# RoboSafe-Lab/Controllable-Latent-Diffusion-for-Traffic-Simulation

Hardware: NVIDIA B200
Metric: guided scenarios/sec (50-step DDIM) (higher is better)
Workload: dtype bf16

## Files before the change

controllable-latent-diffusion-for-traffic-simulation_b200/csrc/cld_api.cu:

```cuda
#include <math.h>
#include <stdarg.h>
#include <stdlib.h>
#include <string.h>

#include "common.cuh"
#include "unet_tc.cuh"

static std::string g_create_err;

namespace cld {

int fail(CldHandle* h, int code, const char* fmt, ...) {
  char buf[512];
  va_list ap;
  va_start(ap, fmt);
  vsnprintf(buf, sizeof(buf), fmt, ap);
  va_end(ap);
  if (h) h->err = buf; else g_create_err = buf;
  return code;
}

int prof_begin(CldHandle* h, int kind, cudaStream_t s) {
  if (!h->profiling) return 0;
  if (h->ev_used + 2 > h->ev_pool.size()) {
// ... 149 lines not shown
    block(2 * lvl + 1);
    if (lvl < 2) conv(u.down[lvl], c.dims[lvl], c.dims[lvl], 3, k3, L.down[lvl][0], L.down[lvl][1]);
  }
  for (int lvl = 0; lvl < 2; ++lvl) {
    block(8 + 2 * lvl);
    block(9 + 2 * lvl);
    const int ch = lvl == 0 ? d1 : d0;
    const int iw = L.up[lvl][0] = take((int64_t)ch * ch * 4), ib = L.up[lvl][1] = take(ch);
    pack(u.up[lvl][0], iw, ch, ch, 4, 2, kte, 1);
    pack(u.up[lvl][1], iw, ch, ch, 4, 2, kto, 1);
    job(2, ib, buf(&u.up_b[lvl], ch), ch);
  }
  block(6);
  block(7);
  conv(u.fin0, d0, d0, 5, k5, L.fin[0], L.fin[1]);
  L.fin[2] = vec(&u.fin0n.g, d0);
  L.fin[3] = vec(&u.fin0n.b, d0);
  conv(u.fin1, D, d0, 1, k1, L.fin[4], L.fin[5]);
  if (rc) return rc;
  if (L.numel.size() > (size_t)PACK_MAX_SRC)
    return fail(h, CLD_ERR_UNSUPPORTED, "the denoiser has %zu tensors, the weight pack takes at most %d", L.numel.size(), PACK_MAX_SRC);
  for (PackJob& j : jobs) {
    j.blk0 = h->pack_blocks;
    h->pack_blocks += (j.total + PACK_BLOCK_ELEMS - 1) / PACK_BLOCK_ELEMS;
  }
  h->pack_njobs = (int)jobs.size();
  if ((rc = dev_alloc(h, &h->pack_jobs, jobs.size()))) return rc;
  CLD_CUDA_OK(h, cudaMemcpy(h->pack_jobs, jobs.data(), jobs.size() * sizeof(PackJob), cudaMemcpyHostToDevice));
  CLD_CUDA_OK(h, cudaStreamSynchronize(cudaStreamLegacy));
  return 0;
}

}

using namespace cld;

extern "C" {

int cld_version(void) { return 100; }

const char* cld_last_error(const CldHandle* h) { return h ? h->err.c_str() : g_create_err.c_str(); }

int cld_create(const CldConfig* cfg, CldHandle** out) {
  if (!cfg || !out) return fail(nullptr, CLD_ERR_ARG, "null argument");
  *out = nullptr;
  int dev = 0;
  cudaError_t e = cudaGetDevice(&dev);
  if (e != cudaSuccess) return fail(nullptr, CLD_ERR_CUDA, "cudaGetDevice: %s", cudaGetErrorString(e));
  cudaDeviceProp prop;
  e = cudaGetDeviceProperties(&prop, dev);
  if (e != cudaSuccess) return fail(nullptr, CLD_ERR_CUDA, "cudaGetDeviceProperties: %s", cudaGetErrorString(e));
  if (prop.major != 10)
    return fail(nullptr, CLD_ERR_ARCH, "libcld_b200 requires an sm_100 (B200) device, found sm_%d%d; there is no fallback",
                prop.major, prop.minor);
  if (cfg->horizon % 4 || cfg->horizon < 8 || cfg->horizon > CLD_MAX_T)
    return fail(nullptr, CLD_ERR_ARG, "horizon must be a multiple of 4 in [8,%d]", CLD_MAX_T);
  if (cfg->latent_dim != 4) return fail(nullptr, CLD_ERR_UNSUPPORTED, "latent_dim must be 4");
  if (cfg->base_dim < 2 || cfg->base_dim > 64 || cfg->base_dim % 4)
    return fail(nullptr, CLD_ERR_UNSUPPORTED, "base_dim must be a multiple of 4 in [4,64]");
  for (int i = 0; i < 3; ++i)
    if (cfg->dims[i] % 8 || cfg->dims[i] < 8) return fail(nullptr, CLD_ERR_UNSUPPORTED, "dims must be multiples of 8");
  if (cfg->cond_dim % 4 || cfg->cond_dim < 4) return fail(nullptr, CLD_ERR_UNSUPPORTED, "cond_dim must be a multiple of 4");
  if (cfg->max_rows < 1) return fail(nullptr, CLD_ERR_ARG, "max_rows must be positive");
  if (cfg->n_timesteps < 1) return fail(nullptr, CLD_ERR_ARG, "n_timesteps must be positive");
  {
    TcLevel levels[3];
    const bool t_ok = tc_level_layout(cfg->horizon, levels);
    if (cfg->precision == CLD_PREC_BF16 && !(cfg->dims[0] == 64 && cfg->dims[1] == 128 && cfg->dims[2] == 256 && t_ok && cfg->hidden == 64))
      return fail(nullptr, CLD_ERR_UNSUPPORTED,
                  "the bf16 tensor-core path is built for dims (64,128,256), hidden 64 and a horizon of 16..56 (8 rows per CTA) or 64..104 in "
                  "multiples of 8 (4 rows per CTA as two half-horizon lanes); use precision fp32 for this configuration");
  }
  CldHandle* h = new CldHandle();
  h->cfg = *cfg;
  h->device = dev;
  h->num_sms = prop.multiProcessorCount;
  h->use_lstm_tc = cfg->precision == CLD_PREC_BF16 && cfg->hidden == 64 && getenv("CLD_LSTM_SIMT") == nullptr;
  h->env_lstm_bwd_simt = getenv("CLD_LSTM_BWD_SIMT") != nullptr;
  h->env_guidance_nofork = getenv("CLD_GUIDANCE_NOFORK") != nullptr;
  h->env_lstm_prof = getenv("CLD_LSTM_PROF") != nullptr;
  h->env_map_stats = getenv("CLD_MAP_STATS") != nullptr;
  h->env_map_exhaustive = getenv("CLD_MAP_EXHAUSTIVE") != nullptr;
  h->env_train_serial = getenv("CLD_TRAIN_SERIAL") != nullptr;
  if (const char* e = getenv("CLD_LSTM_PF")) h->env_lstm_pf = atoi(e);
  const int T = cfg->horizon;
  const size_t MR = cfg->max_rows;
  size_t ae = (size_t)T * cfg->dims[0];
  if ((size_t)(T / 2) * cfg->dims[1] > ae) ae = (size_t)(T / 2) * cfg->dims[1];
  if ((size_t)(T / 4) * cfg->dims[2] > ae) ae = (size_t)(T / 4) * cfg->dims[2];
  h->act_elems = ae;
  unet_blocks(h->unet, *cfg);
  const int tb_total = h->unet.tb_total;
  int rc = 0;
  for (int i = 0; i < 7 && !rc; ++i) rc = dev_alloc(h, &h->act[i], MR * ae);
  if (!rc) rc = dev_alloc(h, &h->tcm, MR * (cfg->base_dim + cfg->cond_dim));
  if (!rc) rc = dev_alloc(h, &h->tbias, MR * tb_total);
  if (!rc) rc = dev_alloc(h, &h->tvec, tb_total);
  if (!rc) rc = dev_alloc(h, &h->tvec_all, (size_t)cfg->n_timesteps * tb_total);
  if (!rc) rc = dev_alloc(h, &h->stash, (size_t)2 * T * ((MR + 63) / 64 * 64) * 5 * cfg->hidden);
  if (!rc) rc = dev_alloc(h, &h->ws_act, MR * T * 2);
  if (!rc) rc = dev_alloc(h, &h->ws_h0, MR * cfg->hidden);
  if (!rc) rc = dev_alloc(h, &h->ws_dh0, (size_t)T * MR * cfg->hidden);
  if (!rc) rc = dev_alloc(h, &h->ws_traj, MR * T * 6);
  if (!rc) rc = dev_alloc(h, &h->ws_dtraj, MR * T * 4);
  if (!rc && h->use_lstm_tc) rc = dev_alloc(h, &h->ws_dtraj2, MR * T * 4);
  if (!rc) rc = dev_alloc(h, &h->ws_dacc, MR * T);
  if (!rc) rc = dev_alloc(h, &h->map_work, MR * T + 8);
  if (!rc && cudaMemset(h->map_work, 0, 8 * sizeof(int)) != cudaSuccess) rc = fail(h, CLD_ERR_CUDA, "cudaMemset of the map work list failed");
  if (!rc) rc = dev_alloc(h, &h->ws_loss, 7 * MR);
  if (!rc) rc = dev_alloc(h, &h->ws_eps, MR * T * cfg->latent_dim);
  if (!rc) rc = dev_alloc(h, &h->ws_mean, MR * T * cfg->latent_dim);
  if (!rc) rc = dev_alloc(h, &h->ws_x, MR * T * cfg->latent_dim);
  if (!rc) rc = dev_alloc(h, &h->ws_t, MR);
  if (!rc) rc = unet_setup(h);
  if (rc) {
    g_create_err = h->err;
    cld_destroy(h);
    return rc;
  }
  *out = h;
  return CLD_OK;
}

void cld_destroy(CldHandle* h) {
  if (!h) return;
  tc_destroy(h);
  lstm_tc_destroy(h);
  train_destroy(h);
  train_tc_destroy(h);
  if (h->ev_fork) cudaEventDestroy(h->ev_fork);
  if (h->ev_join) cudaEventDestroy(h->ev_join);
  if (h->ev_tvec) cudaEventDestroy(h->ev_tvec);
  if (h->aux_stream) cudaStreamDestroy(h->aux_stream);
  for (cudaEvent_t e : h->ev_pool) cudaEventDestroy(e);
  for (void* p : h->allocs) cudaFree(p);
  delete h;
}

int cld_load_unet(CldHandle* h, const float* const* p, const int64_t* numels, int n, void* stream) {
  if (!h || !p) return fail(h, CLD_ERR_ARG, "null argument");
  const UnetLayout& L = h->unet_layout;
  if (n != (int)L.numel.size()) return fail(h, CLD_ERR_ARG, "cld_load_unet: expected %zu tensors, got %d", L.numel.size(), n);
  PackSrc src;
  for (int i = 0; i < n; ++i) {
    if (!p[i]) return fail(h, CLD_ERR_ARG, "cld_load_unet: tensor %d is null", i);
    if (numels && numels[i] != L.numel[i])
      return fail(h, CLD_ERR_ARG, "cld_load_unet: tensor %d has %lld elements, expected %lld", i, (long long)numels[i], (long long)L.numel[i]);
    src.p[i] = p[i];
  }
  cudaStream_t s = (cudaStream_t)stream;
  repack_all_kernel<<<h->pack_blocks, 256, 0, s>>>(h->pack_jobs, h->pack_njobs, src);
  CLD_LAUNCH_OK(h, "repack_all_kernel");
  h->tvec_all_valid = false;
  train_invalidate(h);
  int rc;
  if (h->cfg.precision == CLD_PREC_BF16 && (rc = tc_finalize(h, p, s))) return rc;
  h->unet.loaded = true;
  return CLD_OK;
}

int cld_load_decoder(CldHandle* h, const float* const* p, int n, void* stream) {
  if (!h || !p) return fail(h, CLD_ERR_ARG, "null argument");
  if (n != 12) return fail(h, CLD_ERR_ARG, "cld_load_decoder: expected 12 tensors, got %d", n);
  cudaStream_t s = (cudaStream_t)stream;
  const int H = h->cfg.hidden, G = 4 * H, C = h->cfg.cond_dim, D = h->cfg.latent_dim;
  DecoderW& w = h->dec;
  int rc;
// ... 391 lines not shown
```

controllable-latent-diffusion-for-traffic-simulation_b200/csrc/common.cuh:

```cuda
#pragma once
#include <cuda_runtime.h>
#include <cuda_bf16.h>
#include <stdint.h>
#include <stdio.h>
#include <string>
#include <vector>

#include "../../include/cld_b200.h"

#define CLD_MAX_T 128
#define CLD_TB_TOTAL_MAX 4096

namespace cld {

struct ConvW {
  float* w = nullptr;
  float* wt = nullptr;
  float* b = nullptr;
  int cin = 0, cout = 0, ntaps = 0;
};
struct GnW {
  float* g = nullptr;
  float* b = nullptr;
};
// ... 37 lines not shown
  bool loaded = false;
};

}

namespace cld {
struct BlkIdx { int tw, tb, c0w, c0b, g0, b0, c1w, c1b, g1, b1, rw, rb; };
struct UnetLayout {
  std::vector<int64_t> numel;
  int tmlp[4];
  BlkIdx blk[12];
  int down[2][2], up[2][2];
  int fin[6];
};

struct PackJob {
  int kind;
  int src;
  float* dst;
  int cout, cin, K, ntaps, ks[5], ld, off, transposed, total, blk0;
};
}

struct CldHandle {
  CldConfig cfg;
  int device = 0;
  int num_sms = 0;
  std::string err;
  cld::UnetW unet;
  cld::UnetLayout unet_layout;
  cld::DecoderW dec;
  cld::Schedule sched;
  std::vector<void*> allocs;
  float* act[8] = {nullptr};
  size_t act_elems = 0;
  float* tcm = nullptr;
  float* tbias = nullptr;
  float* tvec = nullptr;
  float* tvec_all = nullptr;
  bool tvec_all_valid = false;
  cudaEvent_t ev_tvec = nullptr;
  cudaStream_t tvec_stream = nullptr;
  float* stash = nullptr;
  float* ws_act = nullptr;
  float* ws_h0 = nullptr;
  float* ws_dh0 = nullptr;
  float* ws_traj = nullptr;
  float* ws_dtraj = nullptr;
  float* ws_dtraj2 = nullptr;
  float* ws_dacc = nullptr;
  float* ws_adam_m = nullptr;
  float* ws_adam_v = nullptr;
  int* map_work = nullptr;
  uint8_t* map_bits = nullptr;
  size_t map_bits_bytes = 0;
  const void* screen_src = nullptr;
  const uint8_t* screen_pk = nullptr;
  int screen_agents = 0, screen_h = 0, screen_w = 0, screen_packed = 0, screen_pitch = 0;
  cudaStream_t aux_stream = nullptr;
  cudaEvent_t ev_fork = nullptr, ev_join = nullptr;
  float* ws_loss = nullptr;
  float* ws_eps = nullptr;
  float* ws_mean = nullptr;
  float* ws_x = nullptr;
  int64_t* ws_t = nullptr;
  int dbg_stage = -1;
  float* dbg_out = nullptr;
  unsigned long long launches = 0;
  bool profiling = false;
  std::vector<cudaEvent_t> ev_pool;
  std::vector<int> ev_kind;
  size_t ev_used = 0;
  void* tc = nullptr;
  void* lstm_tc = nullptr;
  bool use_lstm_tc = false;
  void* train = nullptr;
  unsigned long long sched_version = 0;
  cld::PackJob* pack_jobs = nullptr;
  int pack_njobs = 0, pack_blocks = 0;
  void* train_tc = nullptr;
  bool train_tf32 = false;
  bool env_train_serial = false;
  bool env_lstm_bwd_simt = false, env_guidance_nofork = false, env_lstm_prof = false, env_map_stats = false, env_map_exhaustive = false;
  int env_lstm_pf = 3;
};

namespace cld {
__host__ __device__ inline size_t stash_index(int layer, int t, int T, int R, int row, int v, int u) {
  const size_t rblk = (size_t)((R + 63) >> 6) * 8;
  return (((((size_t)layer * T + t) * rblk + (size_t)(row >> 3)) * 5 + v) * 64 + u) * 8 + (row & 7);
}
constexpr int STASH_V_STRIDE = 64 * 8;
int fail(CldHandle* h, int code, const char* fmt, ...);
#define CLD_CUDA_OK(h, expr)                                                                   \
  do {                                                                                         \
    cudaError_t _e = (expr);                                                                   \
    if (_e != cudaSuccess)                                                                     \
      return cld::fail(h, CLD_ERR_CUDA, "%s failed: %s (%s:%d)", #expr, cudaGetErrorString(_e), \
                       __FILE__, __LINE__);                                                    \
  } while (0)
#define CLD_LAUNCH_OK(h, name)                                                             \
  do {                                                                                     \
    cudaError_t _e = cudaGetLastError();                                                   \
    if (_e != cudaSuccess)                                                                 \
      return cld::fail(h, CLD_ERR_CUDA, "launch of %s failed: %s", name, cudaGetErrorString(_e)); \
    if (h) ++(h)->launches;                                                                \
  } while (0)

int prof_begin(CldHandle* h, int kind, cudaStream_t s);
int prof_end(CldHandle* h, cudaStream_t s);
int unet_forward_fp32(CldHandle* h, const float* x, const float* cond, const int64_t* t, float* eps,
                      int R, cudaStream_t s);
int unet_stage_elems(const CldHandle* h, int stage);
int unet_time_bias(CldHandle* h, const float* cond, const int64_t* t, int R, cudaStream_t s);
int unet_time_cond(CldHandle* h, const float* cond, const int64_t* t, int R, cudaStream_t s);
int unet_cond_bias(CldHandle* h, const float* cond, int R, cudaStream_t s);
int unet_time_vec(CldHandle* h, int t, cudaStream_t s);
int unet_time_vec_to(CldHandle* h, int t, float* dst, cudaStream_t s);
int gn_mish_launch(CldHandle* h, const float* in, const GnW& n, const float* tbias, int tb_stride, const float* res, float* out,
                   int T, int C, int R, cudaStream_t s);
int unet_train_forward(CldHandle* h, const float* x, const float* cond, const int64_t* t, float* eps, int R, cudaStream_t s);
int unet_train_backward(CldHandle* h, const float* d_eps, float* const* grads, int n, float* dx_out, int R, cudaStream_t s);
int ppo_head(CldHandle* h, const float* eps, const float* x_t, const float* x_tm1, const int64_t* t, const float* logp_old,
             const float* reward, float baseline, const float* baseline_dev, float clip, float* logp_new, float* loss_out, float* d_eps, int R,
             cudaStream_t s);
int adam_step_dev(CldHandle* h, float* p, const float* g, float* m, float* v, size_t n, const double* lr_dev, long long* step_dev, double b1,
                  double b2, double eps, double wd, cudaStream_t s);
int mse_head(CldHandle* h, const float* eps, const float* noise, float* loss_out, float* d_eps, int R, cudaStream_t s);
int adam_step(CldHandle* h, float* p, const float* g, float* m, float* v, size_t n, double lr, double b1, double b2, double eps, double wd,
              int step, cudaStream_t s);
float* train_deps_buffer(CldHandle* h);
bool tfconv_supported(int c0, int c1, int N, int Tp);
int tfconv_launch(CldHandle* h, const float* in0, int c0, const float* in1, int c1, int Ta, int tstride, int Tp, const float* w, int planes,
                  int ntaps, const int* wtap, const int* toff, const float* bias, float* out, int Tout, int ostride, int ooff, int N, int accum,
                  int R, cudaStream_t s);
bool tfwgrad_supported(int c0, int c1, int cout, int Tp, int R);
int tfwgrad_launch(CldHandle* h, const float* in0, int c0, const float* in1, int c1, int Ta, int a_stride, int Tp, const float* dout, int Td,
                   int d_stride, int d_toff, int cout, int ntaps, const int* toff, float* part, size_t part_floats, int max_splits, int R,
                   int* splits_out, cudaStream_t s);
void train_tc_destroy(CldHandle* h);
void train_destroy(CldHandle* h);
void train_invalidate(CldHandle* h);
int posterior_step(CldHandle* h, const float* x, const float* eps, const float* noise, uint64_t seed,
                   uint64_t seq, uint64_t idx_base, int t, int t_next, int sampler, float* x_out, float* mean_out, int R,
                   cudaStream_t s);
int add_noise(CldHandle* h, const float* mean, const float* noise, uint64_t seed, uint64_t seq, uint64_t idx_base, int t,
              float* x_out, int R, cudaStream_t s);
int philox_fill(CldHandle* h, uint64_t seed, uint64_t seq, uint64_t idx_base, float* out, int R, cudaStream_t s);
int fill_t(CldHandle* h, int64_t* t, int value, int R, cudaStream_t s);
int decode_rollout(CldHandle* h, const float* z, const float* cond, const float* curr, float* act_out,
                   float* traj_out, bool save, int R, cudaStream_t s);
int unicycle(CldHandle* h, const float* curr, const float* u, float* state_out, int R, cudaStream_t s);
struct GuideOpt {
  int iter = 1;
  float* m = nullptr;
  float* v = nullptr;
  float step_size = 0.f;
  float bc2_sqrt = 0.f;
};
int decode_h0(CldHandle* h, const float* cond, float* h0, int R, cudaStream_t s);
int decode_backward_update2(CldHandle* h, const float* z_mean, const float* act, const float* curr, const float* dtraj,
                            const float* dtraj2, const float* dacc, const CldGuidanceConfig* g, const GuideOpt& opt, float* z_out,
                            float* grad_out, int R, cudaStream_t s);
int decode_rollout_h0(CldHandle* h, const float* z, const float* h0, const float* curr, float* act_out, float* traj_out,
                      bool save, int R, cudaStream_t s);
int decode_rollout_h0_tc(CldHandle* h, const float* z, const float* h0, const float* curr, float* act_out, float* traj_out,
                         bool save, int R, cudaStream_t s);
int decode_backward_update_tc(CldHandle* h, const float* z_mean, const float* act, const float* curr, const float* dtraj,
                              const float* dtraj2, const float* dacc, const CldGuidanceConfig* g, const GuideOpt& opt, float* z_out,
                              float* grad_out, int R, cudaStream_t s);
void lstm_tc_destroy(CldHandle* h);
int indicators(CldHandle* h, const float* traj, const CldScene* sc, uint8_t* offroad, float* coll,
               float* reward, int R, cudaStream_t s);
int guidance_loss_grad(CldHandle* h, const float* traj, const CldScene* sc, const CldGuidanceConfig* g,
                       float* dtraj, float* dtraj_map, float* dacc, float* loss, int R, cudaStream_t s);
int guidance_prepare_maps(CldHandle* h, const CldScene* sc, cudaStream_t s);
int decode_backward_update(CldHandle* h, const float* z_mean, const float* act, const float* curr,
                           const float* dtraj, const CldGuidanceConfig* g, float* z_out, float* grad_out,
                           int R, cudaStream_t s);
}
```

controllable-latent-diffusion-for-traffic-simulation_b200/csrc/kernels_lstm_tc.cu:

```cuda
#include <cuda_fp16.h>
#include <stdio.h>
#include <stdlib.h>

#include "common.cuh"
#include "lstm_shared.cuh"
#include "tc_common.cuh"

namespace cld {
using namespace tc;

namespace {
constexpr int LT_RB = 32;
constexpr int LT_H = 64;
constexpr int LT_THREADS = 576;
constexpr int LT_WBLK = 16384;
constexpr int LT_OP = 4096;
constexpr int LF_H0 = 0;
constexpr int LF_H1 = LF_H0 + 4 * LT_OP;
constexpr int LF_Z = LF_H1 + 2 * LT_OP;
constexpr int LF_H1F = LF_Z + 6 * LT_OP;
constexpr int LF_H1P = LT_H + 1;
constexpr int LF_HW = LF_H1F + 2 * LT_RB * LF_H1P * 4;
constexpr int LF_BARS = LF_HW + 2 * LT_H * 4;
constexpr int LF_TMEM = LF_BARS + 8 * 8;
// ... 308 lines not shown
        if (PROF && rec && n1a >= P0 && n1a < P0 + PN) tl[n1a - P0][2] = clock64();
        tc_fence_after();
        const uint32_t d1a = tmem_base + 64u + (uint32_t)((n1a & 1) * 64);
        const uint64_t b_1a = bh0 + (uint64_t)((n1a & 1) * 2 * (LT_OP >> 4));
        if (elect_one()) kblock(d1a, wc + 80u, 64u, b_1a, 4, true);
        __syncwarp();
        if (PROF && rec && n1a >= P0 && n1a < P0 + PN) tl[n1a - P0][3] = clock64();
        ++n1a; progressed = true;
      }
      if (!progressed && clock64() - t_loop > 8000000000ll) {
        if (lane == 0) printf("lstm_tc forward: MMA issuer stuck (block %d, n0 %d n1a %d n1b %d e0 %d e1 %d z %d)\n", (int)blockIdx.x, n0, n1a, n1b, e0_done, e1_done, z_done);
        __trap();
      }
    }
    if (PROF && rec)
      for (int k = 0; k < PN; ++k)
        printf("[fwd prof] mma step %d: M0 %7lld - %7lld | M1a %7lld - %7lld | M1b %7lld - %7lld\n", P0 + k, tl[k][0] - tbase, tl[k][1] - tbase,
               tl[k][2] - tbase, tl[k][3] - tbase, tl[k][4] - tbase, tl[k][5] - tbase);
  } else {
    const int row = row0 + lane;
    const bool valid = row < R;
    const float hb0 = a.h2a_b[0], hb1 = a.h2a_b[1];
    if (lane == 0) { mbar_arrive(bar_z); mbar_arrive(bar_z + 8); mbar_arrive(bar_z + 16); }
    float4 zn = make_float4(0.f, 0.f, 0.f, 0.f);
    if (valid && 3 < T) zn = reinterpret_cast<const float4*>(a.z)[(size_t)row * T + 3];
    const DynParams2& d = a.dyn;
    float px = 0.f, py = 0.f, sp = 0.f, psi = 0.f;
    if (valid) { px = a.curr[(size_t)row * 4 + 0]; py = a.curr[(size_t)row * 4 + 1]; sp = a.curr[(size_t)row * 4 + 2]; psi = a.curr[(size_t)row * 4 + 3]; }
    float vprev = clip2(sp, d.v_lo, d.v_hi);
    for (int s = 1; s <= T; ++s) {
      const int t = s - 1;
      lt_wait(bar_e1, (uint32_t)t & 1u, 20000 + t);
      const float* hf = h1f + (t & 1) * (LT_RB * LF_H1P) + lane * LF_H1P;
      float s0 = hb0, s1 = hb1;
#pragma unroll 16
      for (int k = 0; k < LT_H; ++k) {
        const float hv = hf[k];
        s0 = fmaf(hw[k], hv, s0); s1 = fmaf(hw[LT_H + k], hv, s1);
      }
      __syncwarp();
      if (lane == 0) mbar_arrive(bar_a);
      if (s + 2 < T) {
        const int slot = (s + 2) % 3;
        uint8_t* zt = sm + LF_Z + slot * 2 * LT_OP;
        store_split(zt, lane, 0, zn.x); store_split(zt, lane, 1, zn.y); store_split(zt, lane, 2, zn.z); store_split(zt, lane, 3, zn.w);
        fence_proxy_async();
        __syncwarp();
        if (lane == 0) mbar_arrive(bar_z + 8 * slot);
        zn = make_float4(0.f, 0.f, 0.f, 0.f);
        if (valid && s + 3 < T) zn = reinterpret_cast<const float4*>(a.z)[(size_t)row * T + s + 3];
      }
      if (valid) {
        *reinterpret_cast<float2*>(a.act_out + ((size_t)row * T + t) * 2) = make_float2(s0, s1);
        if (a.traj_out) {
          const float a_raw = __fadd_rn(__fmul_rn(s0, d.a_std), d.a_mean);
          const float w_raw = __fadd_rn(__fmul_rn(s1, d.w_std), d.w_mean);
          const float ac = clip2(a_raw, d.acce_lo, d.acce_hi);
          sp = __fadd_rn(sp, __fmul_rn(ac, d.dt));
          const float vnext = clip2(sp, d.v_lo, d.v_hi);
          const float vbar = __fmul_rn(0.5f, __fadd_rn(vprev, vnext));
          const float ve = fabsf(vprev);
          const float yb = fmaxf(fminf(__fmul_rn(d.max_steer, ve), __fdiv_rn(d.max_yawvel, fmaxf(ve, 0.1f))), 0.1f);
          const float w = clip2(w_raw, -yb, yb);
          px = __fadd_rn(px, __fmul_rn(__fmul_rn(vbar, cosf(psi)), d.dt));
          py = __fadd_rn(py, __fmul_rn(__fmul_rn(vbar, sinf(psi)), d.dt));
          psi = __fadd_rn(psi, __fmul_rn(w, d.dt));
          float* o = a.traj_out + ((size_t)row * T + t) * 6;
          *reinterpret_cast<float2*>(o) = make_float2(px, py);
          *reinterpret_cast<float2*>(o + 2) = make_float2(vnext, psi);
          *reinterpret_cast<float2*>(o + 4) = make_float2(a_raw, w_raw);
          vprev = vnext;
        }
      }
    }
  }
  tc_fence_before();
  __syncthreads();
  if (warp == 16) tmem_dealloc(tmem_base, 512);
}

namespace {
constexpr int LB_THREADS = 576;
constexpr int LBK_DG = 0;
__host__ __device__ constexpr int lbk_scr(int T) {
  return (LT_RB * (T * 6 + 4 * (T + 1)) * 4 > 17 * LT_OP) ? ((LT_RB * (T * 6 + 4 * (T + 1)) * 4 + 1023) / 1024) * 1024 : 17 * LT_OP;
}
__host__ __device__ constexpr int lbk_dact(int T) { return LBK_DG + lbk_scr(T); }
__host__ __device__ constexpr int lbk_scale(int T) { return lbk_dact(T) + LT_RB * T * 2 * 4; }
__host__ __device__ constexpr int lbk_hw(int T) { return lbk_scale(T) + LT_RB * 4; }
__host__ __device__ constexpr int lbk_dzs(int T) { return lbk_hw(T) + 2 * LT_H * 4; }
__host__ __device__ constexpr int lbk_bars(int T) { return lbk_dzs(T) + LT_RB * 4 * 4; }
__host__ __device__ constexpr int lbk_smem(int T) { return lbk_bars(T) + 8 * 8 + 16; }
}

struct BwdTcArgs {
  const float *z_mean, *act, *curr, *dtraj, *stash;
  const float* dacc;
  const float* dtraj2;
  const uint8_t* wblob;
  const float* h2a_w;
  float *z_out, *grad_out;
  int R, T;
  DynParams2 dyn;
  int optimizer; float lr;
  GuideOpt opt;
  int pf;
};

__global__ void lstm_tc_pack_bwd_kernel(uint32_t* __restrict__ out, const float* __restrict__ wih0, const float* __restrict__ whh0,
                                        const float* __restrict__ wih1, const float* __restrict__ whh1) {
  const int idx = blockIdx.x * blockDim.x + threadIdx.x;
  if (idx >= LB_WCOLS * 128) return;
  const int m = idx & 127, c = idx >> 7;
  const int layer = c < 128 ? 1 : 0, cc = c & 127;
  const int grow = (cc >> 5) * LT_H + 2 * (cc & 31);
  const int q = m >> 5, l = m & 31, j = l & 15, is_b = l >> 4, u = 16 * q + j;
  float v[2];
  for (int e = 0; e < 2; ++e) {
    const int gr = grow + e;
    if (!is_b) v[e] = (layer == 0 ? whh0 : whh1)[gr * 64 + u];
    else v[e] = layer == 0 ? (u < 4 ? wih0[gr * 4 + u] : 0.f) : wih1[gr * 64 + u];
  }
  const __half2 h = __floats2half2_rn(v[0], v[1]);
  out[idx] = *reinterpret_cast<const uint32_t*>(&h);
}

__device__ __forceinline__ void tmem_ld16_hilo(uint32_t taddr, float (&o)[16]) {
  uint32_t vh[16], vl[16];
  tmem_ld16(taddr, vh);
  tmem_ld16(taddr + 32, vl);
  tmem_wait_ld();
#pragma unroll
  for (int r = 0; r < 16; ++r) o[r] = fmaf(__uint_as_float(vl[r]), 1.0f / 2048.0f, __uint_as_float(vh[r]));
}

__device__ __forceinline__ void ld8(const float* p, float (&o)[8]) {
  asm volatile("ld.global.v8.f32 {%0,%1,%2,%3,%4,%5,%6,%7}, [%8];"
               : "=f"(o[0]), "=f"(o[1]), "=f"(o[2]), "=f"(o[3]), "=f"(o[4]), "=f"(o[5]), "=f"(o[6]), "=f"(o[7]) : "l"(p) : "memory");
}

template <bool PROF, bool MOM>
__global__ void __launch_bounds__(LB_THREADS, 1) lstm_backward_tc_kernel(const BwdTcArgs a) {
  constexpr int P0 = 20, PN = 4;
  long long tl[PN][4];
  const bool rec = PROF && blockIdx.x == 0 && (threadIdx.x & 31) == 0;
  const long long tbase = PROF ? clock64() : 0;
  (void)tl; (void)rec; (void)tbase;
  extern __shared__ __align__(1024) uint8_t smem_raw[];
  uint8_t* sm = smem_raw + ((1024u - (smem_u32(smem_raw) & 1023u)) & 1023u);
  const int tid = threadIdx.x, warp = tid >> 5, lane = tid & 31;
  const int row0 = blockIdx.x * LT_RB, T = a.T, R = a.R;
  const uint32_t bars = smem_u32(sm + lbk_bars(T));
  const uint32_t bar_m1 = bars, bar_m0 = bars + 16, bar_e1 = bars + 24, bar_e0 = bars + 32, bar_dz = bars + 40, bar_dzfree = bars + 48;
  uint32_t* tmem_slot = reinterpret_cast<uint32_t*>(sm + lbk_bars(T) + 64);
  float* dzs = reinterpret_cast<float*>(sm + lbk_dzs(T));
  float* dact = reinterpret_cast<float*>(sm + lbk_dact(T));
  float* inv_scale = reinterpret_cast<float*>(sm + lbk_scale(T));
  float* hw = reinterpret_cast<float*>(sm + lbk_hw(T));

  {
    float* act_s = reinterpret_cast<float*>(sm + LBK_DG);
    float* dtr_s = act_s + LT_RB * T * 2;
    float* scr_s = dtr_s + LT_RB * T * 4;
    const int nrow = min(LT_RB, R - row0);
    for (int i = tid; i < nrow * T * 2 / 4; i += LB_THREADS)
      reinterpret_cast<float4*>(act_s)[i] = reinterpret_cast<const float4*>(a.act + (size_t)row0 * T * 2)[i];
    for (int i = tid; i < nrow * T; i += LB_THREADS) {
      float4 v = reinterpret_cast<const float4*>(a.dtraj + (size_t)row0 * T * 4)[i];
      if (a.dtraj2) {
        const float4 w = reinterpret_cast<const float4*>(a.dtraj2 + (size_t)row0 * T * 4)[i];
        v.x += w.x; v.y += w.y; v.z += w.z; v.w += w.w;
      }
      reinterpret_cast<float4*>(dtr_s)[i] = v;
    }
    if (tid < 2 * LT_H) hw[tid] = a.h2a_w[tid];
    if (tid == 0) {
      mbar_init(bar_m1, 1); mbar_init(bar_m1 + 8, 1); mbar_init(bar_m0, 1); mbar_init(bar_e1, 8); mbar_init(bar_e0, 8);
      mbar_init(bar_dz, 2); mbar_init(bar_dzfree, 1);
      fence_barrier_init();
    }
    if (warp == 16) { tmem_alloc(smem_u32(tmem_slot), 512); tmem_relinquish(); }
    tc_fence_before();
    __syncthreads();
    tc_fence_after();
    if (warp < 16) load_weights_tmem(reinterpret_cast<const uint32_t*>(a.wblob), LB_WCOLS, *tmem_slot + LB_WCOL0, warp & 3, (warp >> 2) & 3, lane);
    if (tid < LT_RB) {
      float* da = dact + tid * T * 2;
      float sc = 1.f;
      if (row0 + tid < R) {
        unicycle_row_backward2(act_s + tid * T * 2, a.curr + (size_t)(row0 + tid) * 4, dtr_s + tid * T * 4, T, a.dyn,
                               scr_s + tid * 4 * (T + 1), da, a.dacc ? a.dacc + (size_t)(row0 + tid) * T : nullptr);
        float m = 0.f;
        for (int i = 0; i < 2 * T; ++i) m = fmaxf(m, fabsf(da[i]));
        if (m > 0.f && m < 3.0e38f) {
          int e;
          frexpf(m, &e);
          e = max(-100, min(100, e));
          sc = ldexpf(1.f, -e);
        }
        for (int i = 0; i < 2 * T; ++i) da[i] *= sc;
      } else {
        for (int i = 0; i < 2 * T; ++i) da[i] = 0.f;
      }
      inv_scale[tid] = 1.f / sc;
    }
    __syncthreads();
    uint4* dg = reinterpret_cast<uint4*>(sm + LBK_DG);
    for (int i = tid; i < 16 * LT_OP / 16; i += LB_THREADS) dg[i] = make_uint4(0u, 0u, 0u, 0u);
  }
  fence_proxy_async();
  tc_fence_before();
  __syncthreads();
  tc_fence_after();
  const uint32_t tmem_base = *tmem_slot;

  if (warp < 16) {
    const int L = warp < 8 ? 1 : 0;
    const int q = warp & 3, rh = (warp >> 2) & 1, j = lane & 15;
    const bool is_b = lane >= 16;
    const int u = 16 * q + j;
    const int rb = rh * 2 + (is_b ? 1 : 0);
    const int rloc = rb * 8;
    const uint32_t lane_t = tmem_base + ((uint32_t)(q * 32) << 16);
    const float hw0 = hw[u], hw1 = hw[LT_H + u];
    const uint32_t bar_e = L ? bar_e1 : bar_e0;
    uint8_t* dgt = sm + LBK_DG + (L ? 0 : 8 * LT_OP);
    float dcrec[8], cprev[8];
#pragma unroll
    for (int r = 0; r < 8; ++r) dcrec[r] = 0.f;
    for (int i = 0; i <= T; ++i) {
      const int t = T - 1 - i;
      float gi[8], gf[8], gg[8], go[8], cc[8];
      if (a.pf > 0 && (j & 3) == 0 && t - a.pf >= 0) {
#pragma unroll
        for (int v = 0; v < 5; ++v)
          asm volatile("prefetch.global.L2 [%0];" ::"l"(a.stash + stash_index(L, t - a.pf, T, R, row0 + rloc, v, u)));
      }
      if (i < T) {
        ld8(a.stash + stash_index(L, t, T, R, row0 + rloc, 0, u), gi);
        ld8(a.stash + stash_index(L, t, T, R, row0 + rloc, 1, u), gf);
        ld8(a.stash + stash_index(L, t, T, R, row0 + rloc, 2, u), gg);
        ld8(a.stash + stash_index(L, t, T, R, row0 + rloc, 3, u), go);
        ld8(a.stash + stash_index(L, t, T, R, row0 + rloc, 4, u), cc);
        if (t >= 1) ld8(a.stash + stash_index(L, t - 1, T, R, row0 + rloc, 4, u), cprev);
        else {
#pragma unroll
          for (int r = 0; r < 8; ++r) cprev[r] = 0.f;
        }
      }
      if (PROF && rec && i >= P0 && i < P0 + PN) tl[i - P0][0] = clock64();
      float dh[8];
      float v0[16];
#pragma unroll
      for (int r = 0; r < 8; ++r) dh[r] = 0.f;
      if (L == 1) {
        if (i >= T) break;
        if (i >= 1) {
          lt_wait(bar_m1 + 8 * ((i - 1) & 1), (uint32_t)((i - 1) >> 1) & 1u, 31000 + i);
          tc_fence_after();
          float v[16];
          tmem_ld16_hilo(lane_t + (uint32_t)(((i - 1) & 1) * 64 + rh * 16), v);
#pragma unroll
          for (int r = 0; r < 8; ++r) {
            const float x = __shfl_xor_sync(0xffffffffu, v[8 + r], 16);
            dh[r] = is_b ? x : v[r];
          }
        }
#pragma unroll
        for (int r = 0; r < 8; ++r) {
          const float2 da = *reinterpret_cast<const float2*>(dact + ((rloc + r) * T + t) * 2);
          dh[r] = fmaf(hw0, da.x, fmaf(hw1, da.y, dh[r]));
        }
      } else {
        if (i < T) lt_wait(bar_m1 + 8 * (i & 1), (uint32_t)(i >> 1) & 1u, 33000 + i);
        if (i >= 1) {
          lt_wait(bar_m0, (uint32_t)(i - 1) & 1u, 32000 + i);
          tc_fence_after();
          tmem_ld16_hilo(lane_t + (uint32_t)(128 + rh * 16), v0);
        }
        if (i < T) {
          tc_fence_after();
          float v1[16];
          tmem_ld16_hilo(lane_t + (uint32_t)((i & 1) * 64 + rh * 16), v1);
#pragma unroll
          for (int r = 0; r < 8; ++r) {
            const float rec_lo = i >= 1 ? v0[r] : 0.f, rec_hi = i >= 1 ? v0[8 + r] : 0.f;
            const float send = is_b ? v1[r] : rec_hi;
            const float x = __shfl_xor_sync(0xffffffffu, send, 16);
            dh[r] = is_b ? (v1[8 + r] + x) : (rec_lo + x);
          }
        }
      }
      if (PROF && rec && i >= P0 && i < P0 + PN) tl[i - P0][1] = clock64();
      if (i < T) {
      float dgi[8], dgf[8], dgg[8], dgo[8];
#pragma unroll
      for (int r = 0; r < 8; ++r) {
        const float tc = tanhf_(cc[r]);
        const float dc = fmaf(dh[r] * go[r], 1.f - tc * tc, dcrec[r]);
        const float d_i = dc * gg[r] * gi[r] * (1.f - gi[r]);
        const float d_f = dc * cprev[r] * gf[r] * (1.f - gf[r]);
        const float d_g = dc * gi[r] * (1.f - gg[r] * gg[r]);
        const float d_o = dh[r] * tc * go[r] * (1.f - go[r]);
        dcrec[r] = dc * gf[r];
        dgi[r] = d_i; dgf[r] = d_f; dgg[r] = d_g; dgo[r] = d_o;
      }
      store_split8(dgt + 0 * LT_OP, rb, u, dgi, 2048.0f, 4 * LT_OP);
      store_split8(dgt + 1 * LT_OP, rb, u, dgf, 2048.0f, 4 * LT_OP);
      store_split8(dgt + 2 * LT_OP, rb, u, dgg, 2048.0f, 4 * LT_OP);
      store_split8(dgt + 3 * LT_OP, rb, u, dgo, 2048.0f, 4 * LT_OP);
      if (PROF && rec && i >= P0 && i < P0 + PN) tl[i - P0][2] = clock64();
      tc_fence_before();
      fence_proxy_async();
      __syncwarp();
      if (lane == 0) mbar_arrive(bar_e);
      if (PROF && rec && i >= P0 && i < P0 + PN) tl[i - P0][3] = clock64();
      }
      if (L == 0 && q == 0 && i >= 1) {
        if (i >= 2) lt_wait(bar_dzfree, (uint32_t)(i - 2) & 1u, 34000 + i);
        if (is_b && j < 4) {
#pragma unroll
          for (int r = 0; r < 16; ++r) dzs[(rh * 16 + r) * 4 + j] = v0[r];
        }
        __syncwarp();
        if (lane == 0) mbar_arrive(bar_dz);
      }
    }
    if (PROF && rec && (warp == 0 || warp == 8 || warp == 9 || warp == 13))
      for (int k = 0; k < PN; ++k)
        printf("[bwd prof] warp %2d L%d step %d: top %7lld | waits done %7lld | grads done %7lld | arrived %7lld\n", warp, L, P0 + k,
               tl[k][0] - tbase, tl[k][1] - tbase, tl[k][2] - tbase, tl[k][3] - tbase);
  } else if (warp == 16) {
    constexpr uint32_t IDESC = idesc_f16(128, LT_RB);
    const uint32_t dg_u = smem_u32(sm + LBK_DG);
    auto product = [&](const uint32_t a0, const uint64_t b0, const uint32_t d0) {
#pragma unroll
      for (int g = 0; g < 4; ++g) {
#pragma unroll
        for (int k = 0; k < 4; ++k) {
#pragma unroll
          for (int part = 0; part < 2; ++part)
            umma_ts_f16(d0 + (uint32_t)(part * 32), a0 + (uint32_t)(g * 32 + 8 * k), b0 + (uint64_t)((part * 4 + g) * (LT_OP >> 4) + NMAJ_KSTEP * k), IDESC,
                        (g | k) ? 1u : 0u);
        }
      }
    };
    const uint32_t a_l1 = tmem_base + LB_WCOL0, a_l0 = tmem_base + LB_WCOL0 + 128u;
    const uint64_t b_l1 = make_desc_nmaj(dg_u), b_l0 = make_desc_nmaj(dg_u + 8u * LT_OP);
    int n1 = 0, n0 = 0;
    const long long t_loop = clock64();
    while (n0 < T) {
      bool progressed = false;
      if (n1 < T && (n1 < 2 || n0 >= n1 - 1) && mbar_test_wait(bar_e1, (uint32_t)n1 & 1u)) {
        if (PROF && rec && n1 >= P0 && n1 < P0 + PN) tl[n1 - P0][0] = clock64();
        tc_fence_after();
        const uint32_t d1 = tmem_base + (uint32_t)((n1 & 1) * 64), bm = bar_m1 + 8 * (n1 & 1);
        if (elect_one()) { product(a_l1, b_l1, d1); umma_commit(bm); }
        __syncwarp();
        if (PROF && rec && n1 >= P0 && n1 < P0 + PN) tl[n1 - P0][1] = clock64();
        ++n1;
        progressed = true;
      }
      if (n0 < n1 && mbar_test_wait(bar_e0, (uint32_t)n0 & 1u)) {
        if (PROF && rec && n0 + 1 >= P0 && n0 + 1 < P0 + PN) tl[n0 + 1 - P0][2] = clock64();
        tc_fence_after();
        if (elect_one()) { product(a_l0, b_l0, tmem_base + 128u); umma_commit(bar_m0); }
        __syncwarp();
        if (PROF && rec && n0 + 1 >= P0 && n0 + 1 < P0 + PN) tl[n0 + 1 - P0][3] = clock64();
        ++n0;
        progressed = true;
      }
      if (!progressed && clock64() - t_loop > 8000000000ll) {
        if (lane == 0) printf("lstm_tc backward: MMA issuer stuck (block %d, n1 %d, n0 %d)\n", (int)blockIdx.x, n1, n0);
        __trap();
      }
    }
    if (PROF && rec)
      for (int k = 0; k < PN; ++k)
        printf("[bwd prof] mma s %d: e1 ok %7lld | L1 issued %7lld | e0 ok %7lld | L0 issued %7lld\n", P0 + k, tl[k][0] - tbase,
               tl[k][1] - tbase, tl[k][2] - tbase, tl[k][3] - tbase);
  }
  else {
    const int row = row0 + lane;
    const bool valid = row < R;
    const float is = inv_scale[lane], lr = a.lr;
    const bool adam = a.optimizer == CLD_OPT_ADAM;
    const bool mom = MOM && adam, mom_in = mom && a.opt.iter > 1;
    auto upd = [&](float z, float g) {
      float m, vv;
      if (adam) return adam_first_step(z, g, lr, m, vv);
      return z - lr * g;
    };
    auto upd_m = [&](float z, float g, float& m, float& vv) {
      if (mom_in) return adam_next_step(z, g, a.opt.step_size, a.opt.bc2_sqrt, m, vv);
      return adam_first_step(z, g, lr, m, vv);
    };
    const float4* zin = reinterpret_cast<const float4*>(a.z_mean);
    float4* mp = reinterpret_cast<float4*>(a.opt.m);
    float4* vp = reinterpret_cast<float4*>(a.opt.v);
    float4 z = make_float4(0.f, 0.f, 0.f, 0.f), m4 = z, v4 = z;
    if (valid) z = zin[(size_t)row * T + (T - 1)];
    if (valid && mom_in) { m4 = mp[(size_t)row * T + (T - 1)]; v4 = vp[(size_t)row * T + (T - 1)]; }
    for (int i = 1; i <= T; ++i) {
      const int tz = T - i;
      lt_wait(bar_dz, (uint32_t)(i - 1) & 1u, 50000 + i);
      float4 g = reinterpret_cast<const float4*>(dzs)[lane];
      __syncwarp();
      if (lane == 0) mbar_arrive(bar_dzfree);
      g.x *= is; g.y *= is; g.z *= is; g.w *= is;
      const float4 zc = z;
      float4 mn = m4, vn = v4;
      if (valid && tz >= 1) {
        z = zin[(size_t)row * T + tz - 1];
        if (mom_in) { m4 = mp[(size_t)row * T + tz - 1]; v4 = vp[(size_t)row * T + tz - 1]; }
      }
      if (valid) {
        const size_t o = (size_t)row * T + tz;
        if (!mom) {
          reinterpret_cast<float4*>(a.z_out)[o] = make_float4(upd(zc.x, g.x), upd(zc.y, g.y), upd(zc.z, g.z), upd(zc.w, g.w));
        } else {
          float4 zn;
          zn.x = upd_m(zc.x, g.x, mn.x, vn.x); zn.y = upd_m(zc.y, g.y, mn.y, vn.y);
          zn.z = upd_m(zc.z, g.z, mn.z, vn.z); zn.w = upd_m(zc.w, g.w, mn.w, vn.w);
          reinterpret_cast<float4*>(a.z_out)[o] = zn;
          mp[o] = mn; vp[o] = vn;
        }
        if (a.grad_out) reinterpret_cast<float4*>(a.grad_out)[o] = g;
      }
    }
  }
  tc_fence_before();
  __syncthreads();
  if (warp == 16) tmem_dealloc(tmem_base, 512);
}

static int lf_smem_req() { return LF_SMEM + 1024 > LT_MIN_SMEM ? LF_SMEM + 1024 : LT_MIN_SMEM; }
static int lb_smem_req(int T) { return lbk_smem(T) + 1024 > LT_MIN_SMEM ? lbk_smem(T) + 1024 : LT_MIN_SMEM; }

struct LstmTcState {
  uint8_t* wfwd = nullptr;
  uint8_t* wbwd = nullptr;
};

static int lstm_tc_prepare(CldHandle* h, cudaStream_t s) {
  if (h->lstm_tc) return 0;
  DecoderW& w = h->dec;
  LstmTcState* st = new LstmTcState();
  CLD_CUDA_OK(h, cudaMalloc((void**)&st->wfwd, (size_t)LF_WCOLS * 128 * 4));
  h->allocs.push_back(st->wfwd);
  lstm_tc_pack_fwd_kernel<<<(LF_WCOLS * 128 + 255) / 256, 256, 0, s>>>(reinterpret_cast<uint32_t*>(st->wfwd), w.wih0_raw, w.whh0_raw, w.wih1_raw, w.whh1_raw);
  CLD_LAUNCH_OK(h, "lstm_tc_pack_fwd_kernel");
  CLD_CUDA_OK(h, cudaFuncSetAttribute(lstm_decode_tc_kernel<true, false>, cudaFuncAttributeMaxDynamicSharedMemorySize, lf_smem_req()));
  CLD_CUDA_OK(h, cudaFuncSetAttribute(lstm_decode_tc_kernel<false, false>, cudaFuncAttributeMaxDynamicSharedMemorySize, lf_smem_req()));
  CLD_CUDA_OK(h, cudaFuncSetAttribute(lstm_decode_tc_kernel<false, true>, cudaFuncAttributeMaxDynamicSharedMemorySize, lf_smem_req()));
  CLD_CUDA_OK(h, cudaMalloc((void**)&st->wbwd, (size_t)LB_WCOLS * 128 * 4));
  h->allocs.push_back(st->wbwd);
  lstm_tc_pack_bwd_kernel<<<(LB_WCOLS * 128 + 255) / 256, 256, 0, s>>>(reinterpret_cast<uint32_t*>(st->wbwd), w.wih0_raw, w.whh0_raw, w.wih1_raw, w.whh1_raw);
  CLD_LAUNCH_OK(h, "lstm_tc_pack_bwd_kernel");
  if (lbk_smem(h->cfg.horizon) + 1024 > 232448) return fail(h, CLD_ERR_UNSUPPORTED, "horizon too long for the tensor-core LSTM backward");
  CLD_CUDA_OK(h, cudaFuncSetAttribute(lstm_backward_tc_kernel<false, false>, cudaFuncAttributeMaxDynamicSharedMemorySize, lb_smem_req(h->cfg.horizon)));
  CLD_CUDA_OK(h, cudaFuncSetAttribute(lstm_backward_tc_kernel<true, false>, cudaFuncAttributeMaxDynamicSharedMemorySize, lb_smem_req(h->cfg.horizon)));
  CLD_CUDA_OK(h, cudaFuncSetAttribute(lstm_backward_tc_kernel<false, true>, cudaFuncAttributeMaxDynamicSharedMemorySize, lb_smem_req(h->cfg.horizon)));
  h->lstm_tc = st;
  return 0;
}

void lstm_tc_destroy(CldHandle* h) {
  if (h->lstm_tc) { delete reinterpret_cast<LstmTcState*>(h->lstm_tc); h->lstm_tc = nullptr; }
}

int decode_rollout_h0_tc(CldHandle* h, const float* z, const float* h0, const float* curr, float* act_out, float* traj_out,
                         bool save, int R, cudaStream_t s) {
  DecoderW& w = h->dec;
  if (!w.loaded) return fail(h, CLD_ERR_STATE, "decoder weights not loaded");
  if (h->cfg.hidden != LT_H || h->cfg.latent_dim != 4) return fail(h, CLD_ERR_UNSUPPORTED, "decoder kernel is specialised for hidden=64, latent=4");
  int rc;
  if ((rc = lstm_tc_prepare(h, s))) return rc;
  const LstmTcState* st = reinterpret_cast<const LstmTcState*>(h->lstm_tc);
  LstmTcArgs a;
  a.z = z; a.h0 = h0; a.curr = curr; a.wblob = st->wfwd; a.b0 = w.b0; a.b1 = w.b1;
  a.h2a_w = w.h2a_w; a.h2a_b = w.h2a_b; a.act_out = act_out; a.traj_out = traj_out; a.stash = save ? h->stash : nullptr;
  a.R = R; a.T = h->cfg.horizon; a.dyn = make_dyn2(h->cfg);
  const int grid = (R + LT_RB - 1) / LT_RB;
  if (save) lstm_decode_tc_kernel<true, false><<<grid, LT_THREADS, lf_smem_req(), s>>>(a);
  else if (h->env_lstm_prof) lstm_decode_tc_kernel<false, true><<<grid, LT_THREADS, lf_smem_req(), s>>>(a);
  else lstm_decode_tc_kernel<false, false><<<grid, LT_THREADS, lf_smem_req(), s>>>(a);
  CLD_LAUNCH_OK(h, "lstm_decode_tc_kernel");
  return 0;
}


int decode_backward_update_tc(CldHandle* h, const float* z_mean, const float* act, const float* curr, const float* dtraj,
                              const float* dtraj2, const float* dacc, const CldGuidanceConfig* g, const GuideOpt& opt, float* z_out,
                              float* grad_out, int R, cudaStream_t s) {
  int rc;
  if ((rc = lstm_tc_prepare(h, s))) return rc;
  const LstmTcState* st = reinterpret_cast<const LstmTcState*>(h->lstm_tc);
  BwdTcArgs a;
  a.z_mean = z_mean; a.act = act; a.curr = curr; a.dtraj = dtraj; a.dtraj2 = dtraj2; a.dacc = dacc; a.stash = h->stash; a.wblob = st->wbwd;
  a.h2a_w = h->dec.h2a_w; a.z_out = z_out; a.grad_out = grad_out; a.R = R; a.T = h->cfg.horizon; a.dyn = make_dyn2(h->cfg);
  a.optimizer = g->optimizer; a.lr = g->lr; a.opt = opt;
  a.pf = h->env_lstm_pf;
  const int grid = (R + LT_RB - 1) / LT_RB;
  if (opt.m) lstm_backward_tc_kernel<false, true><<<grid, LB_THREADS, lb_smem_req(a.T), s>>>(a);
  else if (h->env_lstm_prof) lstm_backward_tc_kernel<true, false><<<grid, LB_THREADS, lb_smem_req(a.T), s>>>(a);
  else lstm_backward_tc_kernel<false, false><<<grid, LB_THREADS, lb_smem_req(a.T), s>>>(a);
  CLD_LAUNCH_OK(h, "lstm_backward_tc_kernel");
  return 0;
}

}
```

Measured before the change: 4443.

## Stream LSTM backward stash through a TMA bulk-copy ring in shared memory

Replaces per-thread global loads and L2 prefetches of the stashed gate activations in the tensor-core LSTM backward with a three-slot shared-memory ring. The MMA warp fills the ring ahead of time using bulk async copies signalled by full/empty mbarriers, and the compute warps read their chunk from shared memory. The tanh of the cell state is also computed one step early from the carried cprev, so the separate cell-state load goes away. The aim is to hide global-memory latency on the serial recurrence, at the cost of more shared memory, extra barrier handshakes, and the loss of the tunable prefetch-distance knob.

```diff
diff --git a/controllable-latent-diffusion-for-traffic-simulation_b200/csrc/cld_api.cu b/controllable-latent-diffusion-for-traffic-simulation_b200/csrc/cld_api.cu
--- a/controllable-latent-diffusion-for-traffic-simulation_b200/csrc/cld_api.cu
+++ b/controllable-latent-diffusion-for-traffic-simulation_b200/csrc/cld_api.cu
@@ -255,7 +255,6 @@
   h->env_map_stats = getenv("CLD_MAP_STATS") != nullptr;
   h->env_map_exhaustive = getenv("CLD_MAP_EXHAUSTIVE") != nullptr;
   h->env_train_serial = getenv("CLD_TRAIN_SERIAL") != nullptr;
-  if (const char* e = getenv("CLD_LSTM_PF")) h->env_lstm_pf = atoi(e);
   const int T = cfg->horizon;
   const size_t MR = cfg->max_rows;
   size_t ae = (size_t)T * cfg->dims[0];
diff --git a/controllable-latent-diffusion-for-traffic-simulation_b200/csrc/common.cuh b/controllable-latent-diffusion-for-traffic-simulation_b200/csrc/common.cuh
--- a/controllable-latent-diffusion-for-traffic-simulation_b200/csrc/common.cuh
+++ b/controllable-latent-diffusion-for-traffic-simulation_b200/csrc/common.cuh
@@ -143,7 +143,6 @@
   bool train_tf32 = false;
   bool env_train_serial = false;
   bool env_lstm_bwd_simt = false, env_guidance_nofork = false, env_lstm_prof = false, env_map_stats = false, env_map_exhaustive = false;
-  int env_lstm_pf = 3;
 };
 
 namespace cld {
@@ -231,6 +230,7 @@
                               const float* dtraj2, const float* dacc, const CldGuidanceConfig* g, const GuideOpt& opt, float* z_out,
                               float* grad_out, int R, cudaStream_t s);
 void lstm_tc_destroy(CldHandle* h);
+int lstm_tc_bwd_smem(int T);
 int indicators(CldHandle* h, const float* traj, const CldScene* sc, uint8_t* offroad, float* coll,
                float* reward, int R, cudaStream_t s);
 int guidance_loss_grad(CldHandle* h, const float* traj, const CldScene* sc, const CldGuidanceConfig* g,
diff --git a/controllable-latent-diffusion-for-traffic-simulation_b200/csrc/kernels_lstm_tc.cu b/controllable-latent-diffusion-for-traffic-simulation_b200/csrc/kernels_lstm_tc.cu
--- a/controllable-latent-diffusion-for-traffic-simulation_b200/csrc/kernels_lstm_tc.cu
+++ b/controllable-latent-diffusion-for-traffic-simulation_b200/csrc/kernels_lstm_tc.cu
@@ -414,16 +414,30 @@
 namespace {
 constexpr int LB_THREADS = 576;
 constexpr int LBK_DG = 0;
+constexpr int LBK_RING = LBK_DG + 16 * LT_OP;
+constexpr int LBK_NSLOT = 3;
+constexpr int LBK_RB_BYTES = 5 * 64 * 8 * 4;
+constexpr int LBK_SLOT = 4 * LBK_RB_BYTES;
 __host__ __device__ constexpr int lbk_scr(int T) {
-  return (LT_RB * (T * 6 + 4 * (T + 1)) * 4 > 17 * LT_OP) ? ((LT_RB * (T * 6 + 4 * (T + 1)) * 4 + 1023) / 1024) * 1024 : 17 * LT_OP;
+  return (LT_RB * (T * 6 + 4 * (T + 1)) * 4 > LBK_RING + LBK_NSLOT * LBK_SLOT) ? ((LT_RB * (T * 6 + 4 * (T + 1)) * 4 + 1023) / 1024) * 1024
+                                                                                : LBK_RING + LBK_NSLOT * LBK_SLOT;
 }
 __host__ __device__ constexpr int lbk_dact(int T) { return LBK_DG + lbk_scr(T); }
 __host__ __device__ constexpr int lbk_scale(int T) { return lbk_dact(T) + LT_RB * T * 2 * 4; }
 __host__ __device__ constexpr int lbk_hw(int T) { return lbk_scale(T) + LT_RB * 4; }
 __host__ __device__ constexpr int lbk_dzs(int T) { return lbk_hw(T) + 2 * LT_H * 4; }
 __host__ __device__ constexpr int lbk_bars(int T) { return lbk_dzs(T) + LT_RB * 4 * 4; }
-__host__ __device__ constexpr int lbk_smem(int T) { return lbk_bars(T) + 8 * 8 + 16; }
-}
+__host__ __device__ constexpr int lbk_smem(int T) { return lbk_bars(T) + 16 * 8 + 16; }
+__device__ __forceinline__ int lbk_chunk(int L, int i, int T) { return L ? (i ? 2 * i - 1 : 0) : min(2 * i + 2, 2 * T - 1); }
+
+__device__ __forceinline__ void lds8(const float* p, bool b, float (&o)[8]) {
+  const float4 x = *reinterpret_cast<const float4*>(p + (b ? 4 : 0));
+  const float4 y = *reinterpret_cast<const float4*>(p + (b ? 0 : 4));
+  const float4 lo = b ? y : x, hi = b ? x : y;
+  o[0] = lo.x; o[1] = lo.y; o[2] = lo.z; o[3] = lo.w; o[4] = hi.x; o[5] = hi.y; o[6] = hi.z; o[7] = hi.w;
+}
+}
+
 
 struct BwdTcArgs {
   const float *z_mean, *act, *curr, *dtraj, *stash;
@@ -436,7 +450,6 @@
   DynParams2 dyn;
   int optimizer; float lr;
   GuideOpt opt;
-  int pf;
 };
 
 __global__ void lstm_tc_pack_bwd_kernel(uint32_t* __restrict__ out, const float* __restrict__ wih0, const float* __restrict__ whh0,
@@ -484,7 +497,8 @@
   const int row0 = blockIdx.x * LT_RB, T = a.T, R = a.R;
   const uint32_t bars = smem_u32(sm + lbk_bars(T));
   const uint32_t bar_m1 = bars, bar_m0 = bars + 16, bar_e1 = bars + 24, bar_e0 = bars + 32, bar_dz = bars + 40, bar_dzfree = bars + 48;
-  uint32_t* tmem_slot = reinterpret_cast<uint32_t*>(sm + lbk_bars(T) + 64);
+  const uint32_t bar_full = bars + 56, bar_empty = bars + 80;
+  uint32_t* tmem_slot = reinterpret_cast<uint32_t*>(sm + lbk_bars(T) + 128);
   float* dzs = reinterpret_cast<float*>(sm + lbk_dzs(T));
   float* dact = reinterpret_cast<float*>(sm + lbk_dact(T));
   float* inv_scale = reinterpret_cast<float*>(sm + lbk_scale(T));
@@ -509,6 +523,7 @@
     if (tid == 0) {
       mbar_init(bar_m1, 1); mbar_init(bar_m1 + 8, 1); mbar_init(bar_m0, 1); mbar_init(bar_e1, 8); mbar_init(bar_e0, 8);
       mbar_init(bar_dz, 2); mbar_init(bar_dzfree, 1);
+      for (int s = 0; s < LBK_NSLOT; ++s) { mbar_init(bar_full + 8 * s, 1); mbar_init(bar_empty + 8 * s, 8); }
       fence_barrier_init();
     }
     if (warp == 16) { tmem_alloc(smem_u32(tmem_slot), 512); tmem_relinquish(); }
@@ -557,27 +572,19 @@
     const float hw0 = hw[u], hw1 = hw[LT_H + u];
     const uint32_t bar_e = L ? bar_e1 : bar_e0;
     uint8_t* dgt = sm + LBK_DG + (L ? 0 : 8 * LT_OP);
-    float dcrec[8], cprev[8];
+    const float* ring = reinterpret_cast<const float*>(sm + LBK_RING) + (rb * LBK_RB_BYTES + u * 32) / 4;
+    const bool hsw = (lane >> 2) & 1;
+    float dcrec[8], cprev[8], tc[8], omt[8];
 #pragma unroll
     for (int r = 0; r < 8; ++r) dcrec[r] = 0.f;
+    ld8(a.stash + stash_index(L, T - 1, T, R, row0 + rloc, 4, u), cprev);
     for (int i = 0; i <= T; ++i) {
       const int t = T - 1 - i;
-      float gi[8], gf[8], gg[8], go[8], cc[8];
-      if (a.pf > 0 && (j & 3) == 0 && t - a.pf >= 0) {
-#pragma unroll
-        for (int v = 0; v < 5; ++v)
-          asm volatile("prefetch.global.L2 [%0];" ::"l"(a.stash + stash_index(L, t - a.pf, T, R, row0 + rloc, v, u)));
-      }
       if (i < T) {
-        ld8(a.stash + stash_index(L, t, T, R, row0 + rloc, 0, u), gi);
-        ld8(a.stash + stash_index(L, t, T, R, row0 + rloc, 1, u), gf);
-        ld8(a.stash + stash_index(L, t, T, R, row0 + rloc, 2, u), gg);
-        ld8(a.stash + stash_index(L, t, T, R, row0 + rloc, 3, u), go);
-        ld8(a.stash + stash_index(L, t, T, R, row0 + rloc, 4, u), cc);
-        if (t >= 1) ld8(a.stash + stash_index(L, t - 1, T, R, row0 + rloc, 4, u), cprev);
-        else {
-#pragma unroll
-          for (int r = 0; r < 8; ++r) cprev[r] = 0.f;
+#pragma unroll
+        for (int r = 0; r < 8; ++r) {
+          tc[r] = tanhf_(cprev[r]);
+          omt[r] = 1.f - tc[r] * tc[r];
         }
       }
       if (PROF && rec && i >= P0 && i < P0 + PN) tl[i - P0][0] = clock64();
@@ -625,15 +632,29 @@
       }
       if (PROF && rec && i >= P0 && i < P0 + PN) tl[i - P0][1] = clock64();
       if (i < T) {
+      const int ch = lbk_chunk(L, i, T), slot = ch % LBK_NSLOT;
+      lt_wait(bar_full + 8 * slot, (uint32_t)(ch / LBK_NSLOT) & 1u, 35000 + 1000 * L + i);
+      const float* cs = ring + slot * (LBK_SLOT / 4);
+      float gi[8], gf[8], gg[8], go[8];
+      lds8(cs + 0 * STASH_V_STRIDE, hsw, gi);
+      lds8(cs + 1 * STASH_V_STRIDE, hsw, gf);
+      lds8(cs + 2 * STASH_V_STRIDE, hsw, gg);
+      lds8(cs + 3 * STASH_V_STRIDE, hsw, go);
+      if (t >= 1) lds8(cs + 4 * STASH_V_STRIDE, hsw, cprev);
+      else {
+#pragma unroll
+        for (int r = 0; r < 8; ++r) cprev[r] = 0.f;
+      }
+      __syncwarp();
+      if (lane == 0) mbar_arrive(bar_empty + 8 * slot);
       float dgi[8], dgf[8], dgg[8], dgo[8];
 #pragma unroll
       for (int r = 0; r < 8; ++r) {
-        const float tc = tanhf_(cc[r]);
-        const float dc = fmaf(dh[r] * go[r], 1.f - tc * tc, dcrec[r]);
+        const float dc = fmaf(dh[r] * go[r], omt[r], dcrec[r]);
         const float d_i = dc * gg[r] * gi[r] * (1.f - gi[r]);
         const float d_f = dc * cprev[r] * gf[r] * (1.f - gf[r]);
         const float d_g = dc * gi[r] * (1.f - gg[r] * gg[r]);
-        const float d_o = dh[r] * tc * go[r] * (1.f - go[r]);
+        const float d_o = dh[r] * tc[r] * go[r] * (1.f - go[r]);
         dcrec[r] = dc * gf[r];
         dgi[r] = d_i; dgf[r] = d_f; dgg[r] = d_g; dgo[r] = d_o;
       }
@@ -680,9 +701,32 @@
     const uint32_t a_l1 = tmem_base + LB_WCOL0, a_l0 = tmem_base + LB_WCOL0 + 128u;
     const uint64_t b_l1 = make_desc_nmaj(dg_u), b_l0 = make_desc_nmaj(dg_u + 8u * LT_OP);
     int n1 = 0, n0 = 0;
+    int nc = 0;
+    const uint32_t ring_u = smem_u32(sm + LBK_RING);
     const long long t_loop = clock64();
     while (n0 < T) {
       bool progressed = false;
+      if (nc < 2 * T && (nc < LBK_NSLOT || mbar_test_wait(bar_empty + 8 * (nc % LBK_NSLOT), (uint32_t)(nc / LBK_NSLOT - 1) & 1u))) {
+        int L, i;
+        if (nc == 2 * T - 1) { L = 0; i = T - 1; }
+        else if (nc == 0 || (nc & 1)) { L = 1; i = (nc + 1) >> 1; }
+        else { L = 0; i = (nc >> 1) - 1; }
+        const int t = T - 1 - i, slot = nc % LBK_NSLOT;
+        if (elect_one()) {
+          const uint32_t dst = ring_u + (uint32_t)(slot * LBK_SLOT), bar = bar_full + 8 * slot;
+          mbar_arrive_expect_tx(bar, (uint32_t)(t >= 1 ? LBK_SLOT : 4 * 4 * STASH_V_STRIDE * 4));
+#pragma unroll
+          for (int b = 0; b < 4; ++b) {
+            bulk_g2s(dst + (uint32_t)(b * LBK_RB_BYTES), a.stash + stash_index(L, t, T, R, row0 + 8 * b, 0, 0), 4 * STASH_V_STRIDE * 4, bar);
+            if (t >= 1)
+              bulk_g2s(dst + (uint32_t)(b * LBK_RB_BYTES + 4 * STASH_V_STRIDE * 4), a.stash + stash_index(L, t - 1, T, R, row0 + 8 * b, 4, 0),
+                       STASH_V_STRIDE * 4, bar);
+          }
+        }
+        __syncwarp();
+        ++nc;
+        progressed = true;
+      }
       if (n1 < T && (n1 < 2 || n0 >= n1 - 1) && mbar_test_wait(bar_e1, (uint32_t)n1 & 1u)) {
         if (PROF && rec && n1 >= P0 && n1 < P0 + PN) tl[n1 - P0][0] = clock64();
         tc_fence_after();
@@ -767,7 +811,7 @@
 }
 
 static int lf_smem_req() { return LF_SMEM + 1024 > LT_MIN_SMEM ? LF_SMEM + 1024 : LT_MIN_SMEM; }
-static int lb_smem_req(int T) { return lbk_smem(T) + 1024 > LT_MIN_SMEM ? lbk_smem(T) + 1024 : LT_MIN_SMEM; }
+int lstm_tc_bwd_smem(int T) { return lbk_smem(T) + 1024 > LT_MIN_SMEM ? lbk_smem(T) + 1024 : LT_MIN_SMEM; }
 
 struct LstmTcState {
   uint8_t* wfwd = nullptr;
@@ -789,10 +833,10 @@
   h->allocs.push_back(st->wbwd);
   lstm_tc_pack_bwd_kernel<<<(LB_WCOLS * 128 + 255) / 256, 256, 0, s>>>(reinterpret_cast<uint32_t*>(st->wbwd), w.wih0_raw, w.whh0_raw, w.wih1_raw, w.whh1_raw);
   CLD_LAUNCH_OK(h, "lstm_tc_pack_bwd_kernel");
-  if (lbk_smem(h->cfg.horizon) + 1024 > 232448) return fail(h, CLD_ERR_UNSUPPORTED, "horizon too long for the tensor-core LSTM backward");
-  CLD_CUDA_OK(h, cudaFuncSetAttribute(lstm_backward_tc_kernel<false, false>, cudaFuncAttributeMaxDynamicSharedMemorySize, lb_smem_req(h->cfg.horizon)));
-  CLD_CUDA_OK(h, cudaFuncSetAttribute(lstm_backward_tc_kernel<true, false>, cudaFuncAttributeMaxDynamicSharedMemorySize, lb_smem_req(h->cfg.horizon)));
-  CLD_CUDA_OK(h, cudaFuncSetAttribute(lstm_backward_tc_kernel<false, true>, cudaFuncAttributeMaxDynamicSharedMemorySize, lb_smem_req(h->cfg.horizon)));
+  if (lstm_tc_bwd_smem(h->cfg.horizon) > 232448) return fail(h, CLD_ERR_UNSUPPORTED, "horizon too long for the tensor-core LSTM backward");
+  CLD_CUDA_OK(h, cudaFuncSetAttribute(lstm_backward_tc_kernel<false, false>, cudaFuncAttributeMaxDynamicSharedMemorySize, lstm_tc_bwd_smem(h->cfg.horizon)));
+  CLD_CUDA_OK(h, cudaFuncSetAttribute(lstm_backward_tc_kernel<true, false>, cudaFuncAttributeMaxDynamicSharedMemorySize, lstm_tc_bwd_smem(h->cfg.horizon)));
+  CLD_CUDA_OK(h, cudaFuncSetAttribute(lstm_backward_tc_kernel<false, true>, cudaFuncAttributeMaxDynamicSharedMemorySize, lstm_tc_bwd_smem(h->cfg.horizon)));
   h->lstm_tc = st;
   return 0;
 }
@@ -832,11 +876,10 @@
   a.z_mean = z_mean; a.act = act; a.curr = curr; a.dtraj = dtraj; a.dtraj2 = dtraj2; a.dacc = dacc; a.stash = h->stash; a.wblob = st->wbwd;
   a.h2a_w = h->dec.h2a_w; a.z_out = z_out; a.grad_out = grad_out; a.R = R; a.T = h->cfg.horizon; a.dyn = make_dyn2(h->cfg);
   a.optimizer = g->optimizer; a.lr = g->lr; a.opt = opt;
-  a.pf = h->env_lstm_pf;
   const int grid = (R + LT_RB - 1) / LT_RB;
-  if (opt.m) lstm_backward_tc_kernel<false, true><<<grid, LB_THREADS, lb_smem_req(a.T), s>>>(a);
-  else if (h->env_lstm_prof) lstm_backward_tc_kernel<true, false><<<grid, LB_THREADS, lb_smem_req(a.T), s>>>(a);
-  else lstm_backward_tc_kernel<false, false><<<grid, LB_THREADS, lb_smem_req(a.T), s>>>(a);
+  if (opt.m) lstm_backward_tc_kernel<false, true><<<grid, LB_THREADS, lstm_tc_bwd_smem(a.T), s>>>(a);
+  else if (h->env_lstm_prof) lstm_backward_tc_kernel<true, false><<<grid, LB_THREADS, lstm_tc_bwd_smem(a.T), s>>>(a);
+  else lstm_backward_tc_kernel<false, false><<<grid, LB_THREADS, lstm_tc_bwd_smem(a.T), s>>>(a);
   CLD_LAUNCH_OK(h, "lstm_backward_tc_kernel");
   return 0;
 }
```

New measurement: 4484 (median of 6 runs). Within noise of the previous version (+0.9%).
